# pirovc/ganon

Hardware: AMD Instinct MI355X
Metric: Mreads/s classified (150 bp) + IBF-lookup GB/s vs HBM roofline (higher is better)
Workload: dtype u64

## Files before the change

### ganon_amd/csrc/gn_capi.hip

```cpp
#include "gn_internal.h"

#include <hipcub/hipcub.hpp>
#include "gn_scan.h"
#include "gn_screen_table.h"

#include <algorithm>
#include <cstdarg>
#include <cstdio>
#include <cstdlib>
#include <cstring>
#include <mutex>
#include <new>
#include <unordered_map>
#include <vector>

#include <sys/mman.h>

static thread_local char g_err[512] = "";

int gn_fail(int code, const char* fmt, ...)
{
    va_list ap;
    va_start(ap, fmt);
    vsnprintf(g_err, sizeof(g_err), fmt, ap);
// ... 3 lines not shown

extern "C" const char* gn_last_error(void)
{
    return g_err;
}

static GnSwitches g_sw;

static int gn_parse_switches(const char* list, GnSwitches* out, char* bad, size_t bad_len)
{
    GnSwitches sw;
    struct
    {
        const char* name;
        bool GnSwitches::* flag;
    } static const flags[] = {{"early_exit", &GnSwitches::early_exit},       {"row_screen", &GnSwitches::row_screen},       {"cand_select", &GnSwitches::cand_select},
                              {"csr_identity", &GnSwitches::csr_identity},   {"uniform_select", &GnSwitches::uniform_select},
                              {"run_select", &GnSwitches::run_select},       {"max_first", &GnSwitches::max_first},
                              {"const_nb", &GnSwitches::const_nb},           {"split_kernel", &GnSwitches::split_kernel},
                              {"predrop", &GnSwitches::predrop},             {"deferred_grids", &GnSwitches::deferred_grids}, {"on_demand", &GnSwitches::on_demand}, {"hibf_dense_rows", &GnSwitches::hibf_dense_rows},
                              {"hibf_reg", &GnSwitches::hibf_reg},           {"hibf_pack", &GnSwitches::hibf_pack},
                              {"hibf_one_pack", &GnSwitches::hibf_one_pack}, {"gather_copy", &GnSwitches::gather_copy},     {"joint_apart", &GnSwitches::joint_apart},
                              {"pinned_malloc", &GnSwitches::pinned_malloc}, {"inflate_ahead", &GnSwitches::inflate_ahead}, {"debug", &GnSwitches::debug},
                              {"fake_count", &GnSwitches::fake_count}, {"seg_result", &GnSwitches::seg_result}};
    for (const char* p = list ? list : ""; *p;)
    {
        const char* e = strchr(p, ',');
        size_t      n = e ? (size_t)(e - p) : strlen(p);
        while (n && (*p == ' ' || *p == '\t'))
            ++p, --n;
        while (n && (p[n - 1] == ' ' || p[n - 1] == '\t'))
// ... 844 lines not shown
    ok(s->d_off1.alloc((size_t)max_reads + 1));
    ok(s->d_off2.alloc((size_t)max_reads + 1));
    ok(s->d_slot_cnt.alloc((size_t)max_reads + 1));
    ok(s->d_slot_off.alloc((size_t)max_reads + 1));
    ok(s->d_hashes.alloc(max_bases));
    ok(s->d_nh.alloc(max_reads));
    ok(s->d_status.alloc((size_t)max_reads + 8));
    ok(s->d_matches.alloc(s->match_cap));
    ok(s->d_sorted.alloc(s->match_cap));
    ok(s->d_ctr.alloc(GN_NCTR));
    ok(s->d_seg_begin.alloc(nseg));
    ok(s->d_seg_count.alloc(nseg + 1));
    ok(s->d_seg_off.alloc(nseg + 1));
    ok(s->d_deferred.alloc(max_reads));
    ok(s->d_mdeferred.alloc(max_reads));
    size_t tmp1 = 0, tmp2 = 0;
    hipcub::DeviceScan::ExclusiveSum(nullptr, tmp1, s->d_slot_cnt.get(), s->d_slot_off.get(), (int)(max_reads + 1), s->st);
    gn_scan_counts(nullptr, tmp2, s->d_seg_count, s->d_seg_off, (int)(nseg + 1), s->st);
    s->scan_tmp_bytes = std::max(tmp1, tmp2) + 256;
    ok(s->d_scan_tmp.alloc(s->scan_tmp_bytes));
    if (f->is_hibf)
    {
        s->work_cap = max_reads * 4u > 1024u ? max_reads * 4u : 1024u;
        ok(s->d_work[0].alloc(s->work_cap));
        ok(s->d_work[1].alloc(s->work_cap));
        ok(s->d_hdefer.alloc(s->work_cap));
        ok(s->d_hdefer2.alloc(s->work_cap));
        ok(s->d_hctr.alloc(37 * (GN_HIBF_MAXDEPTH + 1) + 2));
        ok(s->d_hsub.alloc(384 * (GN_HIBF_MAXDEPTH + 1)));
        ok(s->h_hctr.alloc(5 * (GN_HIBF_MAXDEPTH + 1) + 2));
// ... 268 lines not shown
                               s->v_status, s->v_nh, lo, hi, (uint32_t)f->geom.wpr, f->n_targets ? f->n_targets : 1u, s->d_ctr);
        GN_HIP(hipGetLastError());
        return GN_OK;
    }
    p.wpr        = f->geom.wpr;
    p.gp_log2    = f->geom.gp_log2;
    p.slice_dwords = f->geom.slice_dwords;
    p.matches    = s->d_matches;
    p.match_cap  = s->match_cap;
    p.cursor     = s->d_ctr;
    p.seg_begin  = s->d_seg_begin;
    p.seg_count  = s->d_seg_count;
    p.dense      = nullptr;
    p.max_blocks = (uint32_t)f->n_cu * 16u;
    p.max_blocks_fast = (uint32_t)f->n_cu * (f->geom.lw == 1 ? 8u : 6u);
    p.emit_probe = gn_sw().emit_probe;
    p.early_exit = gn_sw().early_exit ? 0u : 1u;
    p.skip_ctr   = s->d_ctr + 7;
    if (f->identity && p.early_exit && !gn_sw().row_screen && (f->geom.lw == 1 || p.W > 128))
    {
        uint8_t ds[GN_SCREEN_NMAX + 1];
        gn_screen_table(p.rel_cutoff, f->ibf.h, (uint32_t)std::min<uint64_t>(f->ibf.W, 64u * f->geom.lw) * 64u, ds);
        memcpy(p.screen, ds, sizeof(p.screen));
    }
    if (lo == 0)
        GN_HIP(hipMemsetAsync(s->d_ctr + 7, 0, sizeof(unsigned long long), s->st));
    p.sl_nbr = f->d_sl_nbr;
    p.csr_identity = f->csr_identity && !gn_sw().csr_identity ? 1u : 0u;
    p.uniform_nb   = p.csr_identity && !gn_sw().uniform_select ? f->uniform_nb : 0u;
    p.run_select   = p.csr_identity && f->run_ok && !p.uniform_nb && !gn_sw().run_select ? 1u : 0u;
// ... 25 lines not shown
        GN_HIP(gn_launch_count_split(p, f->geom, f->ibf.h, s->st));
        p.max_blocks = keep;
        p.work_list  = s->d_deferred;
        p.work_count = s->d_ctr + 4;
    }
    if (fast)
    {
        GN_HIP(hipMemsetAsync(s->d_ctr + 4, 0, sizeof(unsigned long long), s->st));
        p.work_list_out  = s->d_deferred;
        p.work_count_out = s->d_ctr + 4;
        if (!gn_sw().on_demand)
        {
            GN_HIP(hipMemsetAsync(s->d_ctr + 72, 0, sizeof(unsigned long long), s->st));
            p.grab = s->d_ctr + 72;
        }
        GN_HIP(gn_launch_count_fast(p, f->geom, f->ibf.h, s->st));
        p.grab       = nullptr;
        p.work_list  = s->d_deferred;
        p.work_count = s->d_ctr + 4;
    }
    if ((fast || split) && s->prev_count_deferred != ~0ull && lo == 0 && hi == s->n_reads && !gn_sw().deferred_grids)
        p.max_blocks = (uint32_t)std::min<uint64_t>(p.max_blocks, std::max<uint64_t>((uint64_t)f->n_cu, s->prev_count_deferred * 2));
    GN_HIP(gn_launch_count(p, f->geom, f->ibf.h, s->st));
    if (s->long_reads)
    {
        GN_HIP(hipMemsetAsync(s->d_long_count, 0, sizeof(unsigned long long), s->st));
        p.work_list = nullptr;
        GN_HIP(gn_launch_count_long(p, f->ibf.h, s->d_long_list, s->d_long_count, s->d_long_scratch, GN_LONG_BLOCKS, s->st));
    }
    return GN_OK;
}
// ... 286 lines not shown
        if (gn_sw().debug)
            fprintf(stderr, "[gn_finish] attempt %d need %llu cap %llu nh %llu\n", attempt, (unsigned long long)need,
                    (unsigned long long)s->match_cap, (unsigned long long)s->h_ctr[1]);
        if (need <= s->match_cap)
        {
            s->n_matches = s->h_ctr[6];
            if (s->pf_on && (!s->pf_joint || s->pf_joint_done))
            {
                if (stale)
                    GN_HIP(hipMemcpy(s->pf.h_ctr, s->pf.d_ctr, 4 * sizeof(unsigned long long), hipMemcpyDeviceToHost));
                s->n_matches = s->pf.h_ctr[2];
            }
            if (!s->f->is_hibf)
            {
                s->prev_count_deferred = s->h_ctr[4];
                if (!s->src)
                    s->prev_min_deferred = s->h_ctr[5];
            }
            return GN_OK;
        }
        const uint64_t ncap = need + need / 8 + 1024, ocap = s->match_cap;
        s->d_matches.reset();
        s->d_sorted.reset();
        if (s->d_matches.alloc(ncap) != hipSuccess || s->d_sorted.alloc(ncap) != hipSuccess)
        {
            (void)hipGetLastError();
            s->d_matches.reset();
            s->d_sorted.reset();
            s->match_cap  = 0;
            s->classified = false;
// ... 252 lines not shown
    tm.n_hashes = 0;
    for (int i = 8; i < 8 + 64; ++i)
        tm.n_hashes += (s->src ? s->src : s)->h_ctr[i];
    tm.n_matches = s->n_matches;
    tm.n_count_launches = s->n_chunks;
    if (s->f->is_hibf)
        tm.algo_bytes = s->h_ctr[2];
    else
        tm.algo_bytes = tm.n_hashes * (uint64_t)s->f->ibf.h * s->f->ibf.W * 8ull;
    tm.fetched_bytes = tm.algo_bytes - (s->f->is_hibf ? 0ull : (uint64_t)s->h_ctr[7]);
    if (s->cmp_timed && hipEventSynchronize(s->ev_cmp[1]) == hipSuccess)
        hipEventElapsedTime(&tm.ms_compact, s->ev_cmp[0], s->ev_cmp[1]);
    *t = tm;
    return GN_OK;
}
```

### ganon_amd/csrc/gn_internal.h

```cpp
#pragma once

#include <hip/hip_runtime.h>
#include <stdint.h>

#include <vector>

#include "../../include/ganon_hip.h"
#include "../../include/ganon_ibf_hash.h"
#include "gn_devmem.h"

#define GN_MAX_CHUNKS 64
#define GN_CAND_NBIG 4u
#define GN_HIBF_MAXDEPTH 64
#define GN_HIBF_TIMED_LEVELS 8
#define GN_PF_MAX_JOINT 16
#define GN_PF_MAX_DEVICES 16
#define GN_LONG_BLOCKS 128u
#define GN_NCTR 73

struct GnSwitches
{
    bool early_exit = false;
    bool row_screen = false;
    bool cand_select = false;
    bool csr_identity = false;
    bool uniform_select = false;
    bool run_select = false;
    bool max_first = false;
    bool const_nb = false;
    bool split_kernel = false;
    bool predrop = false;
    bool deferred_grids = false;
    bool seg_result = false;
    bool on_demand = false;
    bool hibf_reg = false;
    bool hibf_pack = false;
    bool hibf_one_pack = false;
    bool hibf_dense_rows = false;
// ... 58 lines not shown
    double          rel_cutoff;
    uint32_t wpr;
    uint32_t gp_log2;
    uint32_t slice_dwords;
    gn_match*           matches;
    uint64_t            match_cap;
    unsigned long long* cursor;
    uint64_t*           seg_begin;
    uint32_t*           seg_count;
    uint16_t* dense;
    uint32_t  dense_begin, dense_end;
    const uint32_t*           work_list;
    const unsigned long long* work_count;
    uint32_t*                 work_list_out;
    unsigned long long*       work_count_out;
    uint32_t                  max_blocks;
    uint32_t                  max_blocks_fast;
    uint32_t                  emit_probe;
    const uint32_t*           bin_tgt;
    const uint32_t*           bin_nb2;
    uint32_t                  nbtab_off;
    uint32_t                  candcnt_off;
    const uint32_t*           big_list;
    uint32_t                  n_big;
    const uint32_t*           sl_nbr;
    uint32_t                  early_exit;
    unsigned long long*       skip_ctr;
    uint32_t                  screen[32];
    unsigned long long*       grab;
    uint32_t            uniform_nb;
// ... 222 lines not shown
    const uint32_t*     v_nh       = nullptr;
    const uint8_t*      v_status   = nullptr;
    gn_stream*          src        = nullptr;
    GnDev<gn_match>     d_matches;
    GnDev<gn_match>     d_sorted;
    bool                segmented  = false;
    bool                compacted  = true;
    gn_match*           pf_out     = nullptr;
    hipEvent_t          ev_cmp[2]{};
    bool                cmp_timed  = false;
    GnDev<unsigned long long> d_ctr;
    GnDev<uint64_t>     d_seg_begin;
    GnDev<uint32_t>     d_seg_count;
    GnDev<uint64_t>     d_seg_off;
    GnDev<uint32_t>     d_deferred;
    GnDev<uint32_t>     d_mdeferred;
    GnDev<uint8_t>      d_scan_tmp;
    size_t              scan_tmp_bytes = 0;
    GnDev<uint2>  d_work[2];
    GnDev<uint2>  d_hdefer;
    GnDev<uint2>  d_hdefer2;
    GnDev<unsigned long long> d_hsub;
    GnDev<unsigned long long> d_hctr;
    GnPinned<unsigned long long> h_hctr;
    uint32_t      work_cap = 0;
    GnHibfSortBufs sort;
    hipEvent_t    ev_lvl[GN_HIBF_TIMED_LEVELS + 1]{};
    uint32_t      hibf_levels_run = 0;
    uint32_t      hibf_ranges = 0;
    uint32_t      hibf_range_reads = 0;
// ... 12 lines not shown
    bool                pf_merge  = false;
    GnFastqBufs         fq;
    GnFastqMateBufs     fq2;
    GnFastqHdrBufs      fqh;
    uint64_t            fq_bytes = 0;
    uint32_t            fq_reads = 0;
    bool                fq_pair = false;
    double              fq_probe[4]{};
    bool                fq_pending = false;
    GnPinned<unsigned long long> h_ctr;
    uint32_t n_reads = 0;
    uint64_t n_bases = 0;
    bool     paired  = false;
    bool     have_reads = false, classified = false, hashed = false;
    bool     ctr_copied = false;
    uint64_t prev_count_deferred = ~0ull, prev_min_deferred = ~0ull;
    uint32_t k = 0, w = 0;
    double   rel_cutoff = 0;
    uint64_t n_matches = 0;
    gn_timings tm{};
};
```

### ganon_amd/csrc/gn_kernels.hip

```cpp
#include "gn_internal.h"
#include <cstdlib>

#define GN_WAVE 64
#define GN_CAND_LIMIT 128u
#ifndef GN_NARROW_MAX
#define GN_NARROW_MAX 4u
#endif
#define GN_MATCH_CHUNK 256u
#ifndef GN_MATCH_CHUNK_MAX
#define GN_MATCH_CHUNK_MAX 8192u
#endif
#define GN_STAGE_CAP 128u

struct GnRankLut
{
    uint8_t t[256];
    constexpr GnRankLut() : t{}
    {
        for (int i = 0; i < 256; ++i)
            t[i] = 0;
        t['C'] = t['c'] = 1;
        t['G'] = t['g'] = 2;
        t['T'] = t['t'] = t['U'] = t['u'] = 3;
        t['Y'] = t['y'] = 1;
// ... 894 lines not shown
#ifndef GN_FAST_WPE_LW2_H4
#define GN_FAST_WPE_LW2_H4 3
#endif

constexpr uint32_t GN_FAST_EE_GP_LOG2 = 6;
static_assert((1u << GN_FAST_EE_GP_LOG2) == GN_WAVE, "the EE instances of the fast kernel: one hash group a wave");
template <int HF, int LW, bool EE, bool WIDE = false, bool SCRN = false>
__global__ __launch_bounds__(256) __attribute__((amdgpu_waves_per_eu(EE ? (LW == 1 ? GN_FAST_WPE_LW1 : (HF <= 4 && !WIDE ? GN_FAST_WPE_LW2_H4 : GN_FAST_WPE_LW2)) : 1))) void gn_ibf_count_fast_kernel(GnCountParams p)
{
    extern __shared__ __attribute__((aligned(16))) uint32_t gn_lds[];
    constexpr int      ND   = 2 * LW;
    constexpr int      HFP  = HF <= 4 ? 4 : 8;
    constexpr uint32_t NMAX = 127;
    constexpr bool     SCR  = SCRN && EE && HF == 4 && (LW == 1 || WIDE);
    static_assert(SCR == SCRN, "a screening instance: early exit, four hash functions, 8-byte lanes or the wide build");

    const int      lane  = threadIdx.x & (GN_WAVE - 1);
    const int      wave  = __builtin_amdgcn_readfirstlane((int)(threadIdx.x >> 6));
    const uint32_t wpr   = p.wpr;
    const uint32_t gpl   = SCR ? GN_FAST_EE_GP_LOG2 : p.gp_log2;
    const uint32_t Gp    = 1u << gpl;
    const uint32_t H     = GN_WAVE >> gpl;
    const uint32_t gl    = lane & (Gp - 1);
    const uint32_t hsub  = lane >> gpl;
    uint32_t*      rowtab = gn_lds + (size_t)wave * 128 * HFP;
    uint32_t*      mlist  = gn_lds + (size_t)(blockDim.x >> 6) * 128 * HFP + (size_t)wave * GN_FAST_LIST;

    const uint64_t n_units = (uint64_t)(p.n_reads - p.read_begin) * wpr;
    const uint64_t stride  = (uint64_t)gridDim.x * (blockDim.x >> 6);
    uint64_t       unit    = (uint64_t)blockIdx.x * (blockDim.x >> 6) + wave;
    if (unit >= n_units)
        return;
    const bool     dyn      = p.grab != nullptr && n_units >= 64u * stride;
    const uint64_t dyn_from = stride * 16u;
    uint64_t       chunk_end = unit + 1;
    if (dyn)
    {
        unit *= 16u;
        chunk_end = unit + 16u;
    }
    unsigned long long g_next = 0;
    uint32_t           g_size = 16u;
    auto               ask    = [&](uint64_t from) {
// ... 6 lines not shown
    const uint32_t q0_c = (uint32_t)lane / HF, q1_c = ((uint32_t)lane + GN_WAVE) / HF;
    auto hash_of = [&](uint32_t& q0, uint32_t& q1) {
        if constexpr (!SCR)
        {
            q0 = q0_c;
            q1 = q1_c;
            return;
        }
        uint32_t l = (uint32_t)lane;
        if constexpr (SCR)
            asm volatile("" : "+v"(l));
        q0 = l / HF;
        q1 = (l + GN_WAVE) / HF;
    };
    auto load_meta = [&](uint64_t u, uint32_t& rd, uint32_t& nn, uint64_t& so) {
        rd = p.read_begin + (uint32_t)(u / wpr);
        const uint32_t nh = p.n_hashes[rd];
        nn = p.status[rd] == GN_READ_OK ? nh : 0u;
        so = p.slot_off[rd];
    };
    auto load_hashes = [&](uint32_t nn, uint64_t so, uint64_t& h0, uint64_t& h1) {
        h0 = h1 = 0;
        if (nn >= 1 && nn <= NMAX)
        {
            uint32_t q0, q1;
            hash_of(q0, q1);
            if (q0 < nn)
                h0 = p.hashes[so + q0];
            if (q1 < nn)
                h1 = p.hashes[so + q1];
        }
    };
    unsigned long long chunk_base = 0;
    uint32_t           chunk_left = 0, chunk_size = GN_MATCH_CHUNK;
    uint64_t           skipped_bytes = 0;
    uint32_t           n_pre = 0;
    uint32_t read, n;
    uint64_t slot, hA, hB;
    load_meta(unit, read, n, slot);
    load_hashes(n, slot, hA, hB);

    for (;;)
    {
    const uint32_t slice = (uint32_t)(unit - (uint64_t)(read - p.read_begin) * wpr);
    uint64_t unit_n = unit + 1;
    if (unit_n >= chunk_end)
    {
        if (dyn)
        {
            const uint32_t lo32 = (uint32_t)__builtin_amdgcn_readfirstlane((int)(uint32_t)g_next);
            const uint32_t hi32 = (uint32_t)__builtin_amdgcn_readfirstlane((int)(uint32_t)(g_next >> 32));
            unit_n              = dyn_from + (((uint64_t)hi32 << 32) | lo32);
            chunk_end           = unit_n + g_size;
            if (unit_n < n_units)
                ask(unit_n);
        }
        else
        {
            unit_n    = unit + stride;
// ... 679 lines not shown
        break;
    unit = unit_n; read = read_n; n = n_n; slot = slot_n; hA = hA_n; hB = hB_n;
    }
    if (lane == 0 && skipped_bytes)
        atomicAdd(p.skip_ctr, (unsigned long long)skipped_bytes);
    if (p.pre_mode)
    {
#pragma unroll
        for (int off = 32; off > 0; off >>= 1)
            n_pre += (uint32_t)__shfl_xor((int)n_pre, off);
        if (lane == 0 && n_pre)
            atomicAdd(p.pre_ctr, (unsigned long long)n_pre);
    }
}

template <int HF, int LW, int MAXT>
static hipError_t gn_launch_count_one(const GnCountParams& p, const GnCountGeometry& g, hipStream_t st)
{
    uint32_t blocks = (p.n_reads - p.read_begin + g.rpb - 1) / g.rpb;
    if (blocks > p.max_blocks)
        blocks = p.max_blocks;
    (void)hipFuncSetAttribute(reinterpret_cast<const void*>(gn_ibf_count_kernel<HF, LW, MAXT>),
                              hipFuncAttributeMaxDynamicSharedMemorySize, (int)g.lds_bytes);
    hipLaunchKernelGGL((gn_ibf_count_kernel<HF, LW, MAXT>), dim3(blocks), dim3(g.block), g.lds_bytes, st, p);
    return hipGetLastError();
}

template <int HF, int LW>
static hipError_t gn_launch_fast_one(const GnCountParams& p, hipStream_t st)
{
    const bool ee = p.early_exit && p.gp_log2 == GN_FAST_EE_GP_LOG2;
    const uint64_t units  = (uint64_t)(p.n_reads - p.read_begin) * p.wpr;
    uint32_t       blocks = (uint32_t)((units + 3) / 4);
    if (blocks > p.max_blocks_fast)
        blocks = p.max_blocks_fast;
    const size_t   lds    = 4 * (128 * (HF <= 4 ? 4 : 8) + GN_FAST_LIST) * 4;
    bool scr = false;
    if constexpr (HF == 4)
        for (uint32_t w : p.screen)
            scr = scr || w != 0;
    scr = scr && ee;
    if constexpr (HF == 4 && LW == 2)
        if (scr && p.W > 128)
        {
            hipLaunchKernelGGL((gn_ibf_count_fast_kernel<HF, LW, true, true, true>), dim3(blocks), dim3(256), lds, st, p);
            return hipGetLastError();
        }
    if constexpr (HF == 4 && LW == 1)
        if (scr)
        {
            hipLaunchKernelGGL((gn_ibf_count_fast_kernel<HF, LW, true, false, true>), dim3(blocks), dim3(256), lds, st, p);
            return hipGetLastError();
        }
    if (ee && LW == 2 && p.W > 128)
        hipLaunchKernelGGL((gn_ibf_count_fast_kernel<HF, LW, true, LW == 2>), dim3(blocks), dim3(256), lds, st, p);
    else if (ee)
        hipLaunchKernelGGL((gn_ibf_count_fast_kernel<HF, LW, true>), dim3(blocks), dim3(256), lds, st, p);
    else
        hipLaunchKernelGGL((gn_ibf_count_fast_kernel<HF, LW, false>), dim3(blocks), dim3(256), lds, st, p);
    return hipGetLastError();
// ... 188 lines not shown
```

### ganon_amd/hip.py

```python
from __future__ import annotations

import ctypes as C
import os
from typing import Optional, Sequence, Tuple

import numpy as np

_HERE = os.path.dirname(os.path.abspath(__file__))
_LIB_PATH = os.environ.get("GANON_HIP_LIB") or os.path.join(_HERE, "csrc", "libganon_hip.so")

READ_OK, READ_SMALL, READ_BIG = 0, 1, 2
FILL_3_OF_8 = 0x38
FILL_3_OF_16 = 0x3F
MATCH_DTYPE = np.dtype([("read", "<u4"), ("target", "<u4"), ("count", "<u4")])

ABI_SYMBOLS = ["gn_device_count", "gn_last_error", "gn_filter_upload_ibf", "gn_filter_upload_hibf", "gn_filter_emplace",
               "gn_filter_emplace_ibf", "gn_filter_download_rows", "gn_filter_download_row_list", "gn_pinned_alloc",
               "gn_pinned_free", "gn_filter_write_rows", "gn_filter_write_sync", "gn_filter_finalize",
               "gn_filter_fill_random", "gn_filter_info", "gn_filter_free", "gn_stream_create", "gn_stream_destroy",
               "gn_stream_upload_reads", "gn_stream_minimisers", "gn_stream_classify", "gn_submit_batch", "gn_stream_sync", "gn_fetch_batch", "gn_stream_set_postfilter",
               "gn_fetch_postfilter", "gn_streams_postfilter_joint", "gn_stream_set_long_reads", "gn_stream_device_matches",
               "gn_stream_distinct_hashes", "gn_filter_emplace_split", "gn_stream_fetch_hashes", "gn_stream_dense_counts",
               "gn_stream_timings", "gn_gather_create", "gn_gather_create_merged", "gn_gather_run", "gn_gather_fetch", "gn_gather_device_matches",
               "gn_gather_destroy", "gn_device_memory", "gn_hibf_row_stride_words", "gn_gather_run_buffers", "gn_stream_device_offsets", "gn_stream_hibf_levels", "gn_stream_hibf_level_lines", "gn_stream_classify_shared",
               "gn_stream_upload_fastq", "gn_stream_fastq_index", "gn_stream_fastq_keep", "gn_stream_fastq_records",
               "gn_peer_stats", "gn_stream_upload_text", "gn_stream_upload_text_pair", "gn_stream_text_pair_index", "gn_stream_text_pair_records2",
               "gn_ablate", "gn_filter_probe", "gn_reassign_create", "gn_reassign_run", "gn_reassign_diffs", "gn_reassign_fetch", "gn_reassign_info", "gn_reassign_free",
               "gn_inflate_create", "gn_inflate_destroy", "gn_inflate_feed", "gn_inflate_step", "gn_inflate_text", "gn_inflate_text_device",
               "gn_inflate_get_stats", "gn_inflate_cuts", "gn_inflate_set_carry", "gn_stream_upload_text_device", "gn_stream_fastq_headers",
               "gn_inflate_cuts_lines", "gn_inflate_cut_at_lines", "gn_stream_upload_text_pair_device", "gn_stream_fetch_letters",
               "gn_ibf_hash_constants", "gn_inflate_set_turns", "gn_inflate_handoff",
               "gn_stream_upload_text_pair_devices", "gn_hashes_union", "gn_filter_emplace_path", "gn_filter_probe_path", "gn_filter_probe_paths_shared",
               "gn_filter_bin_popcounts", "gn_filter_copy_ibf", "gn_filter_copy_ibf_spans", "gn_filter_fold_ibf", "gn_filter_extend_path",
               "gn_sketches_create", "gn_sketches_free", "gn_sketches_download", "gn_sketches_union_table", "gn_sketches_pair_table"]


class PostFilter(C.Structure):
    _fields_ = [("rel_filter", C.c_double), ("fpr_query", C.c_double), ("target_fpr", C.c_void_p), ("joint", C.c_int),
# ... 119 lines not shown
    L.gn_filter_emplace_path.argtypes = [vp, vp, vp, u32, vp, u32]
    L.gn_filter_probe_path.argtypes = [vp, vp, vp, u32, vp, u32, vp, vp, vp]
    L.gn_filter_probe_paths_shared.argtypes = [vp, vp, u64, vp, u32, u32, vp]
    L.gn_filter_bin_popcounts.argtypes = [vp, u32, vp]
    L.gn_filter_copy_ibf.argtypes = [vp, u32, vp, u32]
    L.gn_filter_copy_ibf_spans.argtypes = [vp, u32, vp, u32, vp, u32]
    L.gn_filter_fold_ibf.argtypes = [vp, u32, u32, u32, vp, u32, vp, u32]
    L.gn_filter_extend_path.argtypes = [vp, vp, vp, u32, vp, u32, vp, vp]
    L.gn_sketches_create.argtypes = [C.c_int, vp, vp, u32, C.POINTER(vp)]
    L.gn_sketches_free.argtypes = [vp]
    L.gn_sketches_download.argtypes = [vp, u32, u32, vp]
    L.gn_sketches_union_table.argtypes = [vp, vp, u32, u32, u32, u32, vp]
    L.gn_sketches_pair_table.argtypes = [vp, vp, u32, vp]
    L.gn_stream_dense_counts.argtypes = [vp, u32, u32, vp]
    L.gn_stream_timings.argtypes = [vp, C.POINTER(Timings)]
    L.gn_gather_create.argtypes = [i32, u32, C.POINTER(vp), vp, C.POINTER(vp)]
    L.gn_gather_create_merged.argtypes = [i32, u32, C.POINTER(vp), vp, C.POINTER(vp)]
    L.gn_gather_run.argtypes = [vp, C.POINTER(vp), u32]
    L.gn_gather_fetch.argtypes = [vp, vp, vp, u64, C.POINTER(u64)]
    L.gn_gather_device_matches.argtypes = [vp, C.POINTER(vp), C.POINTER(vp), C.POINTER(u64), C.POINTER(u64)]
    L.gn_gather_destroy.argtypes = [vp]
    L.gn_gather_run_buffers.argtypes = [vp, C.POINTER(vp), C.POINTER(vp), vp, u32, u32]
    L.gn_stream_device_offsets.argtypes = [vp, C.POINTER(vp)]
    L.gn_ablate.argtypes = [C.c_char_p]
    L.gn_filter_probe.argtypes = [vp, vp, u64, vp, u32, C.POINTER(u64), C.POINTER(u64), C.POINTER(u64)]
    L.gn_stream_hibf_levels.argtypes = [vp, C.POINTER(u32), vp, vp, vp, vp, u32]
    L.gn_stream_hibf_level_lines.argtypes = [vp, vp, u32]
    L.gn_device_memory.argtypes = [i32, C.POINTER(u64), C.POINTER(u64)]
    L.gn_ibf_hash_constants.argtypes = [vp, C.POINTER(u64)]
    L.gn_inflate_set_turns.argtypes = [vp, u32, u32]
# ... 681 lines not shown
        _check(L.gn_stream_fetch_hashes(self._h, _p(ho), _p(hs), len(hs), C.byref(tot)))
        return ho, hs[: int(tot.value)]

    def dense_counts(self, read_begin: int, read_end: int, width: int) -> np.ndarray:
        out = np.zeros((read_end - read_begin, width), dtype=np.uint16)
        _check(load_library().gn_stream_dense_counts(self._h, read_begin, read_end, _p(out)))
        return out

    def timings(self) -> dict:
        t = Timings()
        _check(load_library().gn_stream_timings(self._h, C.byref(t)))
        return dict(ms_minimiser=t.ms_minimiser, ms_count=t.ms_count, ms_total=t.ms_total, n_hashes=t.n_hashes,
                    algo_bytes=t.algo_bytes, n_matches=t.n_matches, n_count_launches=t.n_count_launches,
                    fetched_bytes=t.fetched_bytes, ms_compact=t.ms_compact)

    def hibf_levels(self):
        cap = 8
        n = C.c_uint32(0)
        ms = np.zeros(cap, dtype=np.float32)
        ab = np.zeros(cap, dtype=np.uint64)
        tb = np.zeros(cap, dtype=np.uint64)
        rb = np.zeros(cap, dtype=np.uint32)
        _check(load_library().gn_stream_hibf_levels(self._h, C.byref(n), _p(ms), _p(ab), _p(tb), _p(rb), cap))
        lb = np.zeros(cap, dtype=np.uint64)
        _check(load_library().gn_stream_hibf_level_lines(self._h, _p(lb), cap))
        return [dict(ms=float(ms[i]), algo_bytes=int(ab[i]), table_bytes=int(tb[i]), row_bytes=int(rb[i]), line_bytes=int(lb[i])) for i in range(min(cap, n.value))]

    def destroy(self) -> None:
        if self._h:
            load_library().gn_stream_destroy(self._h)
# ... 8 lines not shown
```

### include/ganon_hip.h

```cpp
#ifndef GANON_HIP_H
#define GANON_HIP_H

#include <stddef.h>
#include <stdint.h>

#ifdef __cplusplus
extern "C" {
#endif

#define GN_OK 0
#define GN_EINVAL (-22)
#define GN_ENOMEM (-12)
#define GN_ENODEV (-19)
#define GN_ERANGE (-34)
#define GN_EOVERFLOW (-75)

typedef struct gn_filter gn_filter;
typedef struct gn_stream gn_stream;

typedef struct
{
    const uint64_t* rows;
    uint64_t        bin_size;
    uint64_t        bin_words;
// ... 182 lines not shown
                       const gn_fold_member* members, uint32_t n_members);

#define GN_SKETCH_M 4096u
#define GN_SKETCH_TABLE_MAX (1ull << 24)
typedef struct gn_sketches gn_sketches;
int gn_sketches_create(int device, const uint64_t* const* sets, const uint64_t* sizes, uint32_t n_sets, gn_sketches** out);
int gn_sketches_free(gn_sketches* s);
int gn_sketches_download(gn_sketches* s, uint32_t first, uint32_t n, uint8_t* out);
int gn_sketches_union_table(gn_sketches* s, const uint32_t* order, uint32_t n, uint32_t j0, uint32_t j1, uint32_t width, uint64_t* out);
int gn_sketches_pair_table(gn_sketches* s, const uint32_t* idx, uint32_t m, uint64_t* out);

int gn_stream_fetch_hashes(gn_stream* s, uint64_t* hash_off, uint64_t* hashes, uint64_t cap, uint64_t* n_total);
int gn_stream_dense_counts(gn_stream* s, uint32_t read_begin, uint32_t read_end, uint16_t* counts);

int gn_stream_timings(gn_stream* s, gn_timings* t);
int gn_stream_hibf_levels(gn_stream* s, uint32_t* n_levels, float* ms, uint64_t* algo_bytes, uint64_t* table_bytes,
                          uint32_t* row_bytes, uint32_t cap);

int gn_stream_hibf_level_lines(gn_stream* s, uint64_t* line_bytes, uint32_t cap);

typedef struct gn_inflate gn_inflate;
typedef struct gn_inflate_stats
{
    uint64_t steps, chunks, fixups, markers, members, text_bytes;
    double   ms_decode, ms_chain, ms_resolve, ms_step_wall;
    double   prof_ms[8];
} gn_inflate_stats;
int gn_inflate_create(int device, uint64_t compressed_bytes, uint32_t chunk_bytes, uint64_t step_bytes, gn_inflate** out);
int gn_inflate_destroy(gn_inflate* z);
int gn_inflate_feed(gn_inflate* z, const uint8_t* data, uint64_t n);
// ... 16 lines not shown
```

Baseline: 251.0.

## Split screened fast count into lean screening kernel plus deferred unit-list pass

Adds a lean, lower-register screening kernel for the identity, four-hash, 8-byte-lane IBF case. It handles the common units whose screen resolves the result and appends the hard units (no screen depth, or too many survivors) to a device unit list. The full fast kernel then runs only over that list, with its grid sized from the previous batch's deferred count. The aim is higher occupancy and less work in the heavy kernel. The cost is an extra launch, an atomic-appended list, and some units whose screening work is done twice.

```diff
diff --git a/ganon_amd/csrc/gn_capi.hip b/ganon_amd/csrc/gn_capi.hip
--- a/ganon_amd/csrc/gn_capi.hip
+++ b/ganon_amd/csrc/gn_capi.hip
@@ -41,7 +41,7 @@
     {
         const char* name;
         bool GnSwitches::* flag;
-    } static const flags[] = {{"early_exit", &GnSwitches::early_exit},       {"row_screen", &GnSwitches::row_screen},       {"cand_select", &GnSwitches::cand_select},
+    } static const flags[] = {{"early_exit", &GnSwitches::early_exit},       {"row_screen", &GnSwitches::row_screen},       {"lean_screen", &GnSwitches::lean_screen},     {"cand_select", &GnSwitches::cand_select},
                               {"csr_identity", &GnSwitches::csr_identity},   {"uniform_select", &GnSwitches::uniform_select},
                               {"run_select", &GnSwitches::run_select},       {"max_first", &GnSwitches::max_first},
                               {"const_nb", &GnSwitches::const_nb},           {"split_kernel", &GnSwitches::split_kernel},
@@ -916,6 +916,8 @@
     ok(s->d_seg_off.alloc(nseg + 1));
     ok(s->d_deferred.alloc(max_reads));
     ok(s->d_mdeferred.alloc(max_reads));
+    if (!f->is_hibf && f->identity && f->ibf.h == 4 && f->geom.lw == 1 && (uint64_t)nseg <= 0xFFFFFFFFull)
+        ok(s->d_unit_list.alloc(nseg ? nseg : 1));
     size_t tmp1 = 0, tmp2 = 0;
     hipcub::DeviceScan::ExclusiveSum(nullptr, tmp1, s->d_slot_cnt.get(), s->d_slot_off.get(), (int)(max_reads + 1), s->st);
     gn_scan_counts(nullptr, tmp2, s->d_seg_count, s->d_seg_off, (int)(nseg + 1), s->st);
@@ -1214,6 +1216,8 @@
     p.dense      = nullptr;
     p.max_blocks = (uint32_t)f->n_cu * 16u;
     p.max_blocks_fast = (uint32_t)f->n_cu * (f->geom.lw == 1 ? 8u : 6u);
+    p.max_blocks_lean = (uint32_t)f->n_cu * 10u;
+    p.max_blocks_list = p.max_blocks_fast;
     p.emit_probe = gn_sw().emit_probe;
     p.early_exit = gn_sw().early_exit ? 0u : 1u;
     p.skip_ctr   = s->d_ctr + 7;
@@ -1269,7 +1273,16 @@
             GN_HIP(hipMemsetAsync(s->d_ctr + 72, 0, sizeof(unsigned long long), s->st));
             p.grab = s->d_ctr + 72;
         }
+        if (s->d_unit_list && !gn_sw().lean_screen)
+        {
+            GN_HIP(hipMemsetAsync(s->d_ctr + 73, 0, sizeof(unsigned long long), s->st));
+            p.unit_list_out  = s->d_unit_list;
+            p.unit_count_out = s->d_ctr + 73;
+            if (s->prev_unit_deferred != ~0ull && lo == 0 && hi == s->n_reads && !gn_sw().deferred_grids)
+                p.max_blocks_list = (uint32_t)std::min<uint64_t>(p.max_blocks_list, std::max<uint64_t>((uint64_t)f->n_cu, s->prev_unit_deferred / 2 + 1));
+        }
         GN_HIP(gn_launch_count_fast(p, f->geom, f->ibf.h, s->st));
+        p.unit_list_out = nullptr;
         p.grab       = nullptr;
         p.work_list  = s->d_deferred;
         p.work_count = s->d_ctr + 4;
@@ -1586,6 +1599,7 @@
             if (!s->f->is_hibf)
             {
                 s->prev_count_deferred = s->h_ctr[4];
+                s->prev_unit_deferred  = s->h_ctr[73];
                 if (!s->src)
                     s->prev_min_deferred = s->h_ctr[5];
             }
@@ -1868,3 +1882,14 @@
     *t = tm;
     return GN_OK;
 }
+
+extern "C" int gn_stream_screen_deferred(gn_stream* s, uint64_t* units)
+{
+    if (!s || !units)
+        return gn_fail(GN_EINVAL, "null argument");
+    int rc = gn_finish(s);
+    if (rc)
+        return rc;
+    *units = s->f->is_hibf ? 0ull : (uint64_t)s->h_ctr[73];
+    return GN_OK;
+}
diff --git a/ganon_amd/csrc/gn_internal.h b/ganon_amd/csrc/gn_internal.h
--- a/ganon_amd/csrc/gn_internal.h
+++ b/ganon_amd/csrc/gn_internal.h
@@ -16,12 +16,13 @@
 #define GN_PF_MAX_JOINT 16
 #define GN_PF_MAX_DEVICES 16
 #define GN_LONG_BLOCKS 128u
-#define GN_NCTR 73
+#define GN_NCTR 74
 
 struct GnSwitches
 {
     bool early_exit = false;
     bool row_screen = false;
+    bool lean_screen = false;
     bool cand_select = false;
     bool csr_identity = false;
     bool uniform_select = false;
@@ -110,6 +111,12 @@
     const unsigned long long* work_count;
     uint32_t*                 work_list_out;
     unsigned long long*       work_count_out;
+    const uint32_t*           unit_list;
+    const unsigned long long* unit_count;
+    uint32_t*                 unit_list_out;
+    unsigned long long*       unit_count_out;
+    uint32_t                  max_blocks_lean;
+    uint32_t                  max_blocks_list;
     uint32_t                  max_blocks;
     uint32_t                  max_blocks_fast;
     uint32_t                  emit_probe;
@@ -362,6 +369,7 @@
     GnDev<uint32_t>     d_seg_count;
     GnDev<uint64_t>     d_seg_off;
     GnDev<uint32_t>     d_deferred;
+    GnDev<uint32_t>     d_unit_list;
     GnDev<uint32_t>     d_mdeferred;
     GnDev<uint8_t>      d_scan_tmp;
     size_t              scan_tmp_bytes = 0;
@@ -404,7 +412,7 @@
     bool     paired  = false;
     bool     have_reads = false, classified = false, hashed = false;
     bool     ctr_copied = false;
-    uint64_t prev_count_deferred = ~0ull, prev_min_deferred = ~0ull;
+    uint64_t prev_count_deferred = ~0ull, prev_min_deferred = ~0ull, prev_unit_deferred = ~0ull;
     uint32_t k = 0, w = 0;
     double   rel_cutoff = 0;
     uint64_t n_matches = 0;
diff --git a/ganon_amd/csrc/gn_kernels.hip b/ganon_amd/csrc/gn_kernels.hip
--- a/ganon_amd/csrc/gn_kernels.hip
+++ b/ganon_amd/csrc/gn_kernels.hip
@@ -932,6 +932,7 @@
     constexpr uint32_t NMAX = 127;
     constexpr bool     SCR  = SCRN && EE && HF == 4 && (LW == 1 || WIDE);
     static_assert(SCR == SCRN, "a screening instance: early exit, four hash functions, 8-byte lanes or the wide build");
+    constexpr bool     LST  = EE && !SCRN && !WIDE && HF == 4 && LW == 1;
 
     const int      lane  = threadIdx.x & (GN_WAVE - 1);
     const int      wave  = __builtin_amdgcn_readfirstlane((int)(threadIdx.x >> 6));
@@ -944,7 +945,10 @@
     uint32_t*      rowtab = gn_lds + (size_t)wave * 128 * HFP;
     uint32_t*      mlist  = gn_lds + (size_t)(blockDim.x >> 6) * 128 * HFP + (size_t)wave * GN_FAST_LIST;
 
-    const uint64_t n_units = (uint64_t)(p.n_reads - p.read_begin) * wpr;
+    uint64_t       n_units = (uint64_t)(p.n_reads - p.read_begin) * wpr;
+    if constexpr (LST)
+        if (p.unit_list)
+            n_units = *p.unit_count;
     const uint64_t stride  = (uint64_t)gridDim.x * (blockDim.x >> 6);
     uint64_t       unit    = (uint64_t)blockIdx.x * (blockDim.x >> 6) + wave;
     if (unit >= n_units)
@@ -981,6 +985,9 @@
         q1 = (l + GN_WAVE) / HF;
     };
     auto load_meta = [&](uint64_t u, uint32_t& rd, uint32_t& nn, uint64_t& so) {
+        if constexpr (LST)
+            if (p.unit_list)
+                u = p.unit_list[u];
         rd = p.read_begin + (uint32_t)(u / wpr);
         const uint32_t nh = p.n_hashes[rd];
         nn = p.status[rd] == GN_READ_OK ? nh : 0u;
@@ -1009,7 +1016,11 @@
 
     for (;;)
     {
-    const uint32_t slice = (uint32_t)(unit - (uint64_t)(read - p.read_begin) * wpr);
+    uint64_t unit_id = unit;
+    if constexpr (LST)
+        if (p.unit_list)
+            unit_id = p.unit_list[unit];
+    const uint32_t slice = (uint32_t)(unit_id - (uint64_t)(read - p.read_begin) * wpr);
     uint64_t unit_n = unit + 1;
     if (unit_n >= chunk_end)
     {
@@ -1719,6 +1730,412 @@
     }
 }
 
+#ifndef GN_FAST_WPE_LEAN
+#define GN_FAST_WPE_LEAN 5
+#endif
+__global__ __launch_bounds__(256) __attribute__((amdgpu_waves_per_eu(GN_FAST_WPE_LEAN))) void gn_ibf_count_fast_kernel_lean(GnCountParams p)
+{
+    extern __shared__ __attribute__((aligned(16))) uint32_t gn_lds[];
+    constexpr int      HF   = 4;
+    constexpr int      ND   = 2;
+    constexpr uint32_t NMAX = 127;
+
+    const int      lane   = threadIdx.x & (GN_WAVE - 1);
+    const int      wave   = __builtin_amdgcn_readfirstlane((int)(threadIdx.x >> 6));
+    const uint32_t wpr    = p.wpr;
+    uint32_t*      rowtab = gn_lds + (size_t)wave * 128 * HF;
+
+    const uint64_t n_units = (uint64_t)(p.n_reads - p.read_begin) * wpr;
+    const uint64_t stride  = (uint64_t)gridDim.x * (blockDim.x >> 6);
+    uint64_t       unit    = (uint64_t)blockIdx.x * (blockDim.x >> 6) + wave;
+    if (unit >= n_units)
+        return;
+    const bool     dyn      = p.grab != nullptr && n_units >= 64u * stride;
+    const uint64_t dyn_from = stride * 16u;
+    uint64_t       chunk_end = unit + 1;
+    if (dyn)
+    {
+        unit *= 16u;
+        chunk_end = unit + 16u;
+    }
+    unsigned long long g_next = 0;
+    uint32_t           g_size = 16u;
+    auto               ask    = [&](uint64_t from) {
+        g_size = from < n_units - n_units / 4u ? 16u : (from < n_units - n_units / 16u ? 8u : 4u);
+        if (lane == 0)
+            g_next = atomicAdd(p.grab, (unsigned long long)g_size);
+    };
+    if (dyn)
+        ask(unit);
+    auto hash_of = [&](uint32_t& q0, uint32_t& q1) {
+        uint32_t l = (uint32_t)lane;
+        asm volatile("" : "+v"(l));
+        q0 = l / HF;
+        q1 = (l + GN_WAVE) / HF;
+    };
+    auto load_meta = [&](uint64_t u, uint32_t& rd, uint32_t& nn, uint64_t& so) {
+        uint32_t w = wpr;
+        asm volatile("" : "+s"(w));
+        rd = p.read_begin + (uint32_t)(u / w);
+        const uint32_t nh = p.n_hashes[rd];
+        nn = p.status[rd] == GN_READ_OK ? nh : 0u;
+        so = p.slot_off[rd];
+    };
+    auto load_hashes = [&](uint32_t nn, uint64_t so, uint64_t& h0, uint64_t& h1) {
+        h0 = h1 = 0;
+        if (nn >= 1 && nn <= NMAX)
+        {
+            uint32_t q0, q1;
+            hash_of(q0, q1);
+            if (q0 < nn)
+                h0 = p.hashes[so + q0];
+            if (q1 < nn)
+                h1 = p.hashes[so + q1];
+        }
+    };
+    unsigned long long chunk_base = 0;
+    uint32_t           chunk_left = 0, chunk_size = GN_MATCH_CHUNK;
+    uint64_t           skipped_bytes = 0;
+    uint32_t read, n;
+    uint64_t slot, hA, hB;
+    load_meta(unit, read, n, slot);
+    load_hashes(n, slot, hA, hB);
+
+    for (;;)
+    {
+    const uint32_t slice = (uint32_t)(unit - (uint64_t)(read - p.read_begin) * wpr);
+    uint64_t unit_n = unit + 1;
+    if (unit_n >= chunk_end)
+    {
+        if (dyn)
+        {
+            const uint32_t lo32 = (uint32_t)__builtin_amdgcn_readfirstlane((int)(uint32_t)g_next);
+            const uint32_t hi32 = (uint32_t)__builtin_amdgcn_readfirstlane((int)(uint32_t)(g_next >> 32));
+            unit_n              = dyn_from + (((uint64_t)hi32 << 32) | lo32);
+            chunk_end           = unit_n + g_size;
+            if (unit_n < n_units)
+                ask(unit_n);
+        }
+        else
+        {
+            unit_n    = unit + stride;
+            chunk_end = unit_n + 1;
+        }
+    }
+    const bool more = unit_n < n_units;
+    uint32_t   read_n = 0, n_n = 0;
+    uint64_t   slot_n = 0, hA_n = 0, hB_n = 0;
+
+    const bool skip = n > NMAX || n == 0;
+    uint32_t   T = 0, ds = 0;
+    if (!skip)
+    {
+        T = (uint32_t)(uint64_t)ceil(__dmul_rn((double)n, p.rel_cutoff));
+        if (T == 0)
+            T = 1;
+        if (p.early_exit && T >= 2)
+        {
+            ds = (p.screen[n >> 2] >> (8u * (n & 3u))) & 0xFFu;
+            if (ds > n || ds + T <= n)
+                ds = 0;
+        }
+    }
+    if (skip || ds == 0)
+    {
+        if (lane == 0)
+        {
+            if (skip)
+            {
+                if (n > NMAX && slice == 0)
+                    p.work_list_out[atomicAdd(p.work_count_out, 1ULL)] = read;
+                uint32_t zero = 0;
+                asm volatile("" : "+v"(zero));
+                p.seg_begin[(size_t)read * wpr + slice] = zero;
+                p.seg_count[(size_t)read * wpr + slice] = zero;
+            }
+            else
+                p.unit_list_out[atomicAdd(p.unit_count_out, 1ULL)] = (uint32_t)unit;
+        }
+        if (!more)
+            break;
+        load_meta(unit_n, read_n, n_n, slot_n);
+        load_hashes(n_n, slot_n, hA_n, hB_n);
+        unit = unit_n; read = read_n; n = n_n; slot = slot_n; hA = hA_n; hB = hB_n;
+        continue;
+    }
+    const uint32_t wi      = slice * 64 + (uint32_t)lane;
+    const bool     col_act = wi < p.W;
+
+    gn_wave_lds_sync();
+    {
+        uint32_t q0, q1;
+        hash_of(q0, q1);
+        if ((uint32_t)lane < n * HF)
+            rowtab[(uint32_t)lane] = gn_ibf_row(hA, (uint32_t)lane - q0 * HF, p.shift, p.S);
+        if ((uint32_t)lane + GN_WAVE < n * HF)
+            rowtab[(uint32_t)lane + GN_WAVE] = gn_ibf_row(hB, (uint32_t)lane + GN_WAVE - q1 * HF, p.shift, p.S);
+        for (uint32_t idx = (uint32_t)lane + 2 * GN_WAVE; idx < n * HF; idx += GN_WAVE)
+        {
+            const uint32_t q = idx / HF, i = idx - q * HF;
+            rowtab[idx] = gn_ibf_row(p.hashes[slot + q], i, p.shift, p.S);
+        }
+    }
+    gn_wave_lds_sync();
+
+    uint32_t nib[ND][4];
+    uint32_t byt[ND][4][2];
+#pragma unroll
+    for (int d = 0; d < ND; ++d)
+#pragma unroll
+        for (int j = 0; j < 4; ++j)
+        {
+            nib[d][j]    = 0;
+            byt[d][j][0] = 0;
+            byt[d][j][1] = 0;
+        }
+    uint32_t acc_n = 0;
+    auto spill_nibbles = [&]() {
+#pragma unroll
+        for (int d = 0; d < ND; ++d)
+#pragma unroll
+            for (int j = 0; j < 4; ++j)
+            {
+                byt[d][j][0] += nib[d][j] & 0x0F0F0F0Fu;
+                byt[d][j][1] += (nib[d][j] >> 4) & 0x0F0F0F0Fu;
+                nib[d][j] = 0;
+            }
+    };
+    const uint32_t wi_ld = col_act ? wi : 0u;
+    auto issue = [&](uint32_t it, GnRowRegs<HF, 1>& R) {
+        uint32_t row[HF];
+#pragma unroll
+        for (int i = 0; i < HF; ++i)
+        {
+            const uint32_t qs = 2 * it + (uint32_t)(i >> 1) < ds ? 2 * it + (uint32_t)(i >> 1) : 2 * it;
+            row[i]            = rowtab[qs * HF + (uint32_t)(i & 1)];
+        }
+#pragma unroll
+        for (int i = 0; i < HF; ++i)
+        {
+            const uint2 v = *reinterpret_cast<const uint2*>(p.rows + ((uint64_t)row[i] * p.W + wi_ld));
+            R.m[i][0] = v.x;
+            R.m[i][1] = v.y;
+        }
+    };
+    auto consume = [&](const GnRowRegs<HF, 1>& R, uint32_t it) {
+        const uint32_t on = col_act ? 0xFFFFFFFFu : 0u, on2 = 2 * it + 1 < ds ? on : 0u;
+#pragma unroll
+        for (int d = 0; d < ND; ++d)
+        {
+            const uint32_t a = R.m[0][d] & R.m[1][d] & on, b = R.m[2][d] & R.m[3][d] & on2;
+#pragma unroll
+            for (int j = 0; j < 4; ++j)
+                nib[d][j] += ((a >> j) & 0x11111111u) + ((b >> j) & 0x11111111u);
+        }
+        acc_n += 2;
+        if (acc_n >= 14)
+        {
+            spill_nibbles();
+            acc_n = 0;
+        }
+    };
+    GnRowRegs<HF, 1> A, Bq;
+    issue(0, A);
+    if (more)
+        load_meta(unit_n, read_n, n_n, slot_n);
+    {
+        const uint32_t its = (ds + 1) >> 1;
+        uint32_t       it  = 0;
+        for (; it + 2 < its; it += 2)
+        {
+            issue(it + 1, Bq);
+            consume(A, it);
+            issue(it + 2, A);
+            consume(Bq, it + 1);
+        }
+        const bool two = it + 1 < its;
+        if (two)
+            issue(it + 1, Bq);
+        consume(A, it);
+        if (two)
+            consume(Bq, it + 1);
+    }
+    if (acc_n)
+        spill_nibbles();
+    uint32_t sm[ND];
+    uint32_t left = 0;
+    {
+        const uint32_t Kt    = (0x80u - (T - (n - ds))) * 0x01010101u;
+        uint32_t       any_t = 0;
+#pragma unroll
+        for (int d = 0; d < ND; ++d)
+        {
+            uint32_t m = 0;
+#pragma unroll
+            for (int j = 0; j < 4; ++j)
+#pragma unroll
+                for (int pp = 0; pp < 2; ++pp)
+                {
+                    const uint32_t g = (byt[d][j][pp] + Kt) & 0x80808080u;
+                    any_t |= g;
+                    m |= (g >> 7) << (4 * pp + j);
+                }
+            sm[d] = m;
+        }
+        if (__ballot(any_t != 0) != 0)
+        {
+            uint32_t c = 0;
+#pragma unroll
+            for (int d = 0; d < ND; ++d)
+                c += (uint32_t)__popc(sm[d]);
+            for (int off = 32; off > 0; off >>= 1)
+                c += __shfl_xor(c, off);
+            left = (uint32_t)__builtin_amdgcn_readfirstlane((int)c);
+        }
+    }
+    const uint32_t wcol = slice * 64 < p.W ? (p.W - slice * 64 < 64u ? p.W - slice * 64 : 64u) : 0u;
+    if (more)
+        load_hashes(n_n, slot_n, hA_n, hB_n);
+    if (left > GN_NARROW_MAX)
+    {
+        if (lane == 0)
+            p.unit_list_out[atomicAdd(p.unit_count_out, 1ULL)] = (uint32_t)unit;
+        skipped_bytes -= (uint64_t)(2 * ds) * wcol * 8ull;
+        if (!more)
+            break;
+        unit = unit_n; read = read_n; n = n_n; slot = slot_n; hA = hA_n; hB = hB_n;
+        continue;
+    }
+    uint32_t narrow_loads = 0;
+    uint32_t total = 0;
+    uint32_t rec_t = 0, rec_c = 0;
+    if (left)
+    {
+        constexpr uint32_t QPC = GN_WAVE / HF;
+        uint64_t           grp = 0;
+#pragma unroll
+        for (uint32_t q = 0; q < QPC; ++q)
+            grp |= 1ULL << (q * HF);
+        const uint32_t l_q = (uint32_t)lane / HF, l_i = (uint32_t)lane - l_q * HF;
+        uint64_t       lm  = __ballot((sm[0] | sm[1]) != 0);
+        while (lm)
+        {
+            const int L = __builtin_ctzll(lm);
+            lm &= lm - 1;
+#pragma unroll
+            for (int d = 0; d < ND; ++d)
+            {
+                uint32_t mb = (uint32_t)__builtin_amdgcn_readlane((int)sm[d], L);
+                while (mb)
+                {
+                    const uint32_t bit = (uint32_t)__builtin_ctz(mb);
+                    mb &= mb - 1;
+                    const uint32_t word = slice * 64 + (uint32_t)L;
+                    const uint32_t sh   = 32u * d + bit;
+                    uint32_t       c2   = 0;
+#pragma unroll
+                    for (int j = 0; j < 4; ++j)
+#pragma unroll
+                        for (int pp = 0; pp < 2; ++pp)
+                            if ((bit & 3u) == (uint32_t)j && ((bit >> 2) & 1u) == (uint32_t)pp)
+                                c2 = byt[d][j][pp];
+                    c2 = ((uint32_t)__builtin_amdgcn_readlane((int)c2, L) >> (8u * (bit >> 3))) & 0xFFu;
+                    uint32_t add     = 0;
+                    uint32_t q_known = ds;
+                    uint32_t q_to    = n;
+                    bool     probe   = c2 != ds;
+                    if (probe)
+                        q_to = ds;
+                    for (;;)
+                    {
+                        add = 0;
+                        for (uint32_t q0 = 0; q0 < q_to; q0 += 2 * QPC)
+                        {
+                            const uint32_t qa = q0 + l_q, qb = qa + QPC;
+                            const bool     ina = qa < q_to, inb = qb < q_to;
+                            uint64_t       wa = ~0ULL, wb = ~0ULL;
+                            if (ina && !(l_i < 2 && qa < q_known))
+                                wa = p.rows[(uint64_t)rowtab[qa * HF + l_i] * p.W + word];
+                            if (inb && !(l_i < 2 && qb < q_known))
+                                wb = p.rows[(uint64_t)rowtab[qb * HF + l_i] * p.W + word];
+                            const uint64_t bma = __ballot(ina && ((wa >> sh) & 1ULL)), bmb = __ballot(inb && ((wb >> sh) & 1ULL));
+                            uint64_t       alla = bma, allb = bmb;
+#pragma unroll
+                            for (int i = 1; i < HF; ++i)
+                            {
+                                alla &= bma >> i;
+                                allb &= bmb >> i;
+                            }
+                            add += (uint32_t)__popcll(alla & grp) + (uint32_t)__popcll(allb & grp);
+                        }
+                        narrow_loads += q_to * HF - 2 * q_known;
+                        if (!probe)
+                            break;
+                        probe = false;
+                        if (add + (n - ds) < T)
+                        {
+                            add = 0;
+                            break;
+                        }
+                        q_known = 0;
+                        q_to    = n;
+                    }
+                    if (add >= T)
+                    {
+                        if ((uint32_t)lane == total)
+                        {
+                            rec_t = word * 64u + sh;
+                            rec_c = add;
+                        }
+                        ++total;
+                    }
+                }
+            }
+        }
+    }
+    if (wcol)
+        skipped_bytes += (uint64_t)(n * HF - 2 * ds) * wcol * 8ull - (uint64_t)narrow_loads * 128ull;
+
+    unsigned long long base = 0;
+    if (total)
+    {
+        if (total > chunk_left)
+        {
+            const uint32_t need = total > chunk_size ? total : chunk_size;
+            chunk_size = chunk_size * 2u <= GN_MATCH_CHUNK_MAX ? chunk_size * 2u : GN_MATCH_CHUNK_MAX;
+            unsigned long long nb = 0;
+            if (lane == 0)
+                nb = atomicAdd(p.cursor, (unsigned long long)need);
+            chunk_base = gn_readlane64(nb, 0);
+            chunk_left = need;
+        }
+        base = chunk_base;
+        chunk_base += total;
+        chunk_left -= total;
+        uint32_t l = (uint32_t)lane;
+        asm volatile("" : "+v"(l));
+        if (base + total <= p.match_cap && l < total)
+        {
+            gn_match mt;
+            mt.read   = read;
+            mt.target = rec_t;
+            mt.count  = rec_c;
+            p.matches[base + l] = mt;
+        }
+    }
+    if (lane == 0)
+    {
+        p.seg_begin[(size_t)read * wpr + slice] = base;
+        p.seg_count[(size_t)read * wpr + slice] = total;
+    }
+    if (!more)
+        break;
+    unit = unit_n; read = read_n; n = n_n; slot = slot_n; hA = hA_n; hB = hB_n;
+    }
+    if (lane == 0 && skipped_bytes)
+        atomicAdd(p.skip_ctr, (unsigned long long)skipped_bytes);
+}
+
 template <int HF, int LW, int MAXT>
 static hipError_t gn_launch_count_one(const GnCountParams& p, const GnCountGeometry& g, hipStream_t st)
 {
@@ -1749,6 +2166,25 @@
         if (scr && p.W > 128)
         {
             hipLaunchKernelGGL((gn_ibf_count_fast_kernel<HF, LW, true, true, true>), dim3(blocks), dim3(256), lds, st, p);
+            return hipGetLastError();
+        }
+    if constexpr (HF == 4 && LW == 1)
+        if (scr && p.unit_list_out != nullptr)
+        {
+            uint32_t lean_blocks = (uint32_t)((units + 3) / 4);
+            if (lean_blocks > p.max_blocks_lean)
+                lean_blocks = p.max_blocks_lean;
+            hipLaunchKernelGGL(gn_ibf_count_fast_kernel_lean, dim3(lean_blocks), dim3(256), 4 * 128 * HF * 4, st, p);
+            hipError_t e = hipGetLastError();
+            if (e != hipSuccess)
+                return e;
+            GnCountParams q = p;
+            q.unit_list     = p.unit_list_out;
+            q.unit_count    = p.unit_count_out;
+            q.grab          = nullptr;
+            if (blocks > p.max_blocks_list)
+                blocks = p.max_blocks_list;
+            hipLaunchKernelGGL((gn_ibf_count_fast_kernel<HF, LW, true>), dim3(blocks ? blocks : 1u), dim3(256), lds, st, q);
             return hipGetLastError();
         }
     if constexpr (HF == 4 && LW == 1)
diff --git a/ganon_amd/hip.py b/ganon_amd/hip.py
--- a/ganon_amd/hip.py
+++ b/ganon_amd/hip.py
@@ -21,7 +21,7 @@
                "gn_stream_upload_reads", "gn_stream_minimisers", "gn_stream_classify", "gn_submit_batch", "gn_stream_sync", "gn_fetch_batch", "gn_stream_set_postfilter",
                "gn_fetch_postfilter", "gn_streams_postfilter_joint", "gn_stream_set_long_reads", "gn_stream_device_matches",
                "gn_stream_distinct_hashes", "gn_filter_emplace_split", "gn_stream_fetch_hashes", "gn_stream_dense_counts",
-               "gn_stream_timings", "gn_gather_create", "gn_gather_create_merged", "gn_gather_run", "gn_gather_fetch", "gn_gather_device_matches",
+               "gn_stream_timings", "gn_stream_screen_deferred", "gn_gather_create", "gn_gather_create_merged", "gn_gather_run", "gn_gather_fetch", "gn_gather_device_matches",
                "gn_gather_destroy", "gn_device_memory", "gn_hibf_row_stride_words", "gn_gather_run_buffers", "gn_stream_device_offsets", "gn_stream_hibf_levels", "gn_stream_hibf_level_lines", "gn_stream_classify_shared",
                "gn_stream_upload_fastq", "gn_stream_fastq_index", "gn_stream_fastq_keep", "gn_stream_fastq_records",
                "gn_peer_stats", "gn_stream_upload_text", "gn_stream_upload_text_pair", "gn_stream_text_pair_index", "gn_stream_text_pair_records2",
@@ -171,6 +171,7 @@
     L.gn_sketches_pair_table.argtypes = [vp, vp, u32, vp]
     L.gn_stream_dense_counts.argtypes = [vp, u32, u32, vp]
     L.gn_stream_timings.argtypes = [vp, C.POINTER(Timings)]
+    L.gn_stream_screen_deferred.argtypes = [vp, C.POINTER(C.c_uint64)]
     L.gn_gather_create.argtypes = [i32, u32, C.POINTER(vp), vp, C.POINTER(vp)]
     L.gn_gather_create_merged.argtypes = [i32, u32, C.POINTER(vp), vp, C.POINTER(vp)]
     L.gn_gather_run.argtypes = [vp, C.POINTER(vp), u32]
@@ -882,6 +883,11 @@
                     algo_bytes=t.algo_bytes, n_matches=t.n_matches, n_count_launches=t.n_count_launches,
                     fetched_bytes=t.fetched_bytes, ms_compact=t.ms_compact)
 
+    def screen_deferred(self) -> int:
+        n = C.c_uint64(0)
+        _check(load_library().gn_stream_screen_deferred(self._h, C.byref(n)))
+        return int(n.value)
+
     def hibf_levels(self):
         cap = 8
         n = C.c_uint32(0)
diff --git a/include/ganon_hip.h b/include/ganon_hip.h
--- a/include/ganon_hip.h
+++ b/include/ganon_hip.h
@@ -220,6 +220,7 @@
 int gn_stream_dense_counts(gn_stream* s, uint32_t read_begin, uint32_t read_end, uint16_t* counts);
 
 int gn_stream_timings(gn_stream* s, gn_timings* t);
+int gn_stream_screen_deferred(gn_stream* s, uint64_t* units);
 int gn_stream_hibf_levels(gn_stream* s, uint32_t* n_levels, float* ms, uint64_t* algo_bytes, uint64_t* table_bytes,
                           uint32_t* row_bytes, uint32_t cap);
 
```

Result: faster. 264.7 (median of 6 runs) (+5.4%).
